# guodashun/peg-in-hole-gym

Hardware: AMD Instinct MI355X
Metric: env-steps/sec (higher is better)
Workload: dtype f32

## Files before the change

### peg_in_hole_gym_amd/csrc/pih_common.h

```cpp
#pragma once
#include <string.h>
#include "../../include/pih.h"
#include "../../include/pih_model.h"
#include "pih_math.h"

namespace pih {

constexpr int NL = PIH_NL, ANL = PIH_ARM_NL, ONL = PIH_OBJ_NL, ND = PIH_NDOF;
constexpr int NSAMP = PIH_PIPE_NSAMP;
constexpr int CMAX = 48;
constexpr int CAMAX = 12;
constexpr int CL = 20;
constexpr int NROWC = 3 * CMAX;
constexpr int WPS = 39;
constexpr int WMS = 31;
constexpr int NMOT = 32;
constexpr int NLIM = 18;
static_assert(PIH_DBG_UDOT + ND <= PIH_DBG_NCONTACT && PIH_DBG_CONTACT + PIH_DBG_CONTACT_STRIDE * CMAX <= PIH_DBG_DINV &&
              PIH_DBG_DINV + 3 * CMAX <= PIH_DBG_CYCLES && PIH_DBG_XCC_ID < PIH_DEBUG_WORDS, "debug words of the peg-in-hole step (include/pih.h PIH_DBG_*) overlap");

PIH_CONST int L_PARENT[NL] = PIH_LINK_PARENT;
PIH_CONST int L_JTYPE[NL] = PIH_LINK_JTYPE;
PIH_CONST real L_RFIX[NL][9] = PIH_LINK_RFIX;
PIH_CONST real L_TFIX[NL][3] = PIH_LINK_TFIX;
PIH_CONST real L_AXIS[NL][3] = PIH_LINK_AXIS;
PIH_CONST real L_MASS[NL] = PIH_LINK_MASS;
PIH_CONST real L_COM[NL][3] = PIH_LINK_COM;
PIH_CONST real L_INERTIA[NL][6] = PIH_LINK_INERTIA;
PIH_CONST real L_LO[NL] = PIH_LINK_LO;
PIH_CONST real L_HI[NL] = PIH_LINK_HI;
PIH_CONST real L_DAMPING[NL] = PIH_LINK_DAMPING;
PIH_CONST real L_MU[NL] = PIH_LINK_MU;
PIH_CONST real ARM_BASE_R[9] = PIH_ARM_BASE_R;
namespace model_ce {
constexpr int JT[NL] = PIH_LINK_JTYPE;
constexpr double DAMP[NL] = PIH_LINK_DAMPING;
constexpr bool structure_ok() {
  for (int L = 0; L < NL; L++) {
    const int want = L < 7 ? PIH_JT_REVOLUTE : (L < ANL ? PIH_JT_PRISMATIC : (L == ANL ? PIH_JT_FLOATING : PIH_JT_REVOLUTE));
    if (JT[L] != want || DAMP[L] != 0.0) return false;
  }
  return true;
}
static_assert(ANL == 9 && structure_ok(), "joint_type() below restates the structure of PIH_LINK_JTYPE / PIH_LINK_DAMPING");
}
PIH_HD int joint_type(int L) { return L < 7 ? PIH_JT_REVOLUTE : (L < ANL ? PIH_JT_PRISMATIC : (L == ANL ? PIH_JT_FLOATING : PIH_JT_REVOLUTE)); }
PIH_CONST real EE_R[9] = PIH_EE_R;
PIH_CONST real EE_T[3] = PIH_EE_T;
PIH_CONST real ARM_REST[9] = PIH_ARM_REST;
PIH_CONST real FBOX_C[2][3] = PIH_FINGER_BOX_C;
PIH_CONST real FBOX_H[3] = PIH_FINGER_BOX_H;
PIH_CONST int ASPH_LINK[PIH_ARM_NSPH] = PIH_ARM_SPH_LINK;
PIH_CONST real ASPH_C[PIH_ARM_NSPH][3] = PIH_ARM_SPH_C;
PIH_CONST real ASPH_R[PIH_ARM_NSPH] = PIH_ARM_SPH_R;
PIH_CONST int SAMP_LINK[NSAMP] = PIH_PIPE_SAMP_LINK;
PIH_CONST real SAMP_Y[NSAMP] = PIH_PIPE_SAMP_Y;
PIH_CONST int SAMP_VERTEX[NSAMP] = PIH_PIPE_SAMP_VERTEX;
PIH_CONST real HOLE_POS[3] = PIH_HOLE_POS;
PIH_CONST real UR5_RFIX[6][9] = PIH_UR5_RFIX;
PIH_CONST real UR5_TFIX[6][3] = PIH_UR5_TFIX;
PIH_CONST real UR5_AXIS[6][3] = PIH_UR5_AXIS;
PIH_CONST real UR5_BASE_T[3] = PIH_UR5_BASE_T;
PIH_CONST real UR5_EE_R[9] = PIH_UR5_EE_R;
PIH_CONST real UR5_EE_T[3] = PIH_UR5_EE_T;
PIH_CONST real IDENT3[9] = {1, 0, 0, 0, 1, 0, 0, 0, 1};
PIH_CONST real ZERO3[3] = {0, 0, 0};
PIH_CONST int FSM_STEPS[10] = PIH_FSM_STEPS;

#define PIH_PI ((real)3.14159265358979323846)
#define PIH_LIN_DAMP ((real)0.04)
#define PIH_ANG_DAMP ((real)0.04)
#define PIH_MAX_COORD_VEL ((real)100)
#define PIH_MAX_FRICTION ((real)10)
#define PIH_BIG ((real)1e30)
#define PIH_MEM_FENCE() __asm__ volatile("" ::: "memory")

#ifdef PIH_AREAL
typedef PIH_AREAL areal;
#else
typedef real areal;
#endif

struct Params {
  real dt, resid, erp, warm, margin, slop, ikdamp, ikres, dv;
  int iters, ikiters, mode, maxsteps, autoreset, selfcol, armcol, debug, env0, pgsmode, attachball, noprio, nospec;
  int object;
  int checkstride;
  uint64_t seed;
};

inline void config_defaults(pih_config* c) {
  memset(c, 0, sizeof *c);
  c->n_envs = 1; c->env_index0 = 0; c->mode = 0; c->solver_iters = 50; c->ik_iters = 20; c->max_episode_steps = 2227; c->auto_reset = 0;
  c->enable_self_collision = 1; c->enable_arm_collision = 3; c->task_id = PIH_TASK_PEG_IN_HOLE; c->debug = 0; c->schedule = 1; c->exit_check_stride = 16;
  c->seed = 0; c->dt = 1.0f / 240.0f; c->residual_threshold = 1e-7f; c->erp = 0.2f; c->warmstart = 0.85f; c->contact_margin = 0.005f;
  c->linear_slop = 1e-5f; c->ik_damping = 0.5f; c->ik_residual = 1e-4f; c->dv = 2.0f / 240.0f;
}
inline Params params_from_config(const pih_config* c) {
  Params P;
  P.dt = (real)c->dt; P.resid = (real)c->residual_threshold; P.erp = (real)c->erp; P.warm = (real)c->warmstart; P.margin = (real)c->contact_margin;
  P.slop = (real)c->linear_slop; P.ikdamp = (real)c->ik_damping; P.ikres = (real)c->ik_residual; P.dv = (real)c->dv;
  P.iters = c->solver_iters; P.ikiters = c->ik_iters; P.mode = c->mode; P.maxsteps = c->max_episode_steps; P.autoreset = c->auto_reset;
  P.selfcol = c->enable_self_collision; P.armcol = c->enable_arm_collision; P.debug = c->debug; P.env0 = c->env_index0; P.seed = c->seed;
  P.pgsmode = c->solver_path; P.attachball = c->attach_ball; P.noprio = (c->schedule & 4) != 0; P.nospec = (c->schedule & 64) != 0;
  P.checkstride = c->exit_check_stride < 1 ? 1 : c->exit_check_stride; P.object = c->object_id;
  return P;
}

template <bool DOUBLED = true, class FC, class FN> PIH_HD int pgs_iteration_loop(int iters, int stride, FC checked, FN unchecked) {
  int it = 0;
  const int lead = stride <= 1 ? iters : 4;
  while (it < iters && it < lead) { it++; if (checked()) return it; }
  while (it < iters) {
    const int stop = it + stride - 1 < iters - 1 ? it + stride - 1 : iters - 1;
    if (DOUBLED) {
      while (it < stop) {
        it++; unchecked();
        if (it >= stop) break;
        it++; unchecked();
      }
    } else {
#pragma nounroll
      while (it < stop) { it++; unchecked(); }
    }
    it++; if (checked()) return it;
  }
  return it;
}

PIH_HD void count_nonfinite_reset(real& rng, real& rng_hi, real& count) {
  rng = (finite_small(rng) && rng >= 0 && rng < (real)16777216) ? rng : (real)0;
  rng_hi = (finite_small(rng_hi) && rng_hi >= 0 && rng_hi < (real)16777216) ? rng_hi : (real)0;
  const real nb = count; count = (finite_small(nb) && nb >= 0 ? nb : (real)0) + 1;
}

PIH_HD int link_dof(int L) { return L < ANL ? L : (L == ANL ? 9 : L + 5); }

constexpr int CREC = 32;
enum : int {
  CR_P = 0,
  CR_LB = 3,
  CR_FLOOR = 4,
  CR_MU = 5,
  CR_ANG = 6,
  CR_PAD = 7,
  CR_DIR0 = 8,
  CR_DINV0 = 11,
  CR_KSTRIDE = 4,
  CR_RHS = 20,
  CR_G = 23,
  CR_LAM = 26,
  CR_DVP_N = CR_LAM,
  CR_THRESH = 29,
  CR_DVP_T1 = CR_THRESH,
};
static_assert(CR_THRESH + 3 == CREC && CR_DINV0 == CR_DIR0 + 3 && CR_DIR0 + 3 * CR_KSTRIDE == CR_RHS && CR_DVP_T1 == CR_DVP_N + 3, "contact record layout");
static_assert(CR_P % 4 == 0 && CR_DIR0 % 4 == 0 && CR_KSTRIDE == 4 && CR_RHS % 4 == 0 && CREC % 4 == 0, "pgs() reads the record as eight real4: (p, lb), (dir k, dinv k) and (rhs, G) each are one 16-byte group");
// ... 523 lines not shown
          else {
            real c = dot(d1, rr);
            if (e <= EPS) { tt = 0; ss = clampr(-c / a, 0, 1); }
            else {
              real b = dot(d1, d2), den = a * e - b * b;
              ss = den > EPS ? clampr((b * f - c * e) / den, 0, 1) : (real)0;
              tt = (b * ss + f) / e;
              if (tt < 0) { tt = 0; ss = clampr(-c / a, 0, 1); } else if (tt > 1) { tt = 1; ss = clampr((b - c) / a, 0, 1); }
            }
          }
          V3 c1 = p1 + ss * d1, c2 = p2 + tt * d2, d = c1 - c2;
          real dist = norm(d); depth = dist - 2 * r;
          if (depth < margin && dist >= (real)1e-9) { n = ((real)1 / dist) * d; p = (real)0.5 * (c1 + c2); valid = true; }
        }
      }
      int slot = w.alloc(valid);
      if (valid && slot < CMAX) emit(slot, ANL + s, ANL + t, 1000 + s * 24 + t, p, n, depth, L_MU[ANL + s] * L_MU[ANL + t]);
    });
  }
  int nc = w.alloc_count(); if (nc > CMAX) nc = CMAX;
  sh.nc = nc; sh.nca = nca;
}

PIH_HD void aba_root_inverse(Shared& sh, const real* Mx, areal* rootp) {
  areal Mq[6][6], Iv[6][6];
  for (int i = 0; i < 6; i++) for (int j = 0; j < 6; j++) { Mq[i][j] = Mx[8 * i + j]; Iv[i][j] = i == j ? (areal)1 : (areal)0; }
#pragma unroll
  for (int k = 0; k < 6; k++) {
    areal pv = (areal)1 / Mq[k][k];
#pragma unroll
    for (int j = 0; j < 6; j++) { Mq[k][j] *= pv; Iv[k][j] *= pv; }
#pragma unroll
    for (int i = 0; i < 6; i++) if (i != k) {
      areal f = Mq[i][k];
#pragma unroll
      for (int j = 0; j < 6; j++) { Mq[i][j] -= f * Mq[k][j]; Iv[i][j] -= f * Iv[k][j]; }
    }
  }
  for (int i = 0; i < 6; i++) { for (int j = 0; j < 6; j++) sh.Inv6[6 * i + j] = (real)Iv[i][j]; rootp[i] = Mx[8 * i + 6]; }
}
PIH_HD int aba_own_word(int i, int j) {
  const int ii = i < 3 ? i : i - 3, jj = j < 3 ? j : j - 3;
  const int sym = ii == jj ? ii : ii + jj + 2;
  if (i >= 6 || j >= 7) return 27;
  if (j == 6) return 21 + i;
  if (i < 3 && j < 3) return sym;
  if (i >= 3 && j >= 3) return 15 + sym;
  if (i < 3) return 6 + 3 * i + jj;
  return 6 + 3 * j + ii;
}
static_assert(NROWC >= 144, "scratch of the inward sweep aliases r_lam");

struct RowOut { real* wa; real* wp; };
PIH_HD real response(const Shared& sh, int la, int lb, V3 p, V3 dir, int jm, RowOut out, V3* dvp_out = nullptr, bool ang = false) {
  real jw = 0; V3 dvp = mk(0, 0, 0);
  bool arm = (la >= 0 && la < ANL) || (lb >= 0 && lb < ANL) || (jm >= 0 && jm < ANL);
  bool obj = (la >= ANL) || (lb >= ANL) || (jm >= ANL);
  if (arm && out.wa) {
    const bool aa_ = la >= 0 && la < ANL, ab_ = lb >= 0 && lb < ANL;
    const V3 rA = p - ld3(sh.LO[aa_ ? la : 0]), rB = p - ld3(sh.LO[ab_ ? lb : 0]);
    const V3 tqa = ang ? dir : cross(rA, dir), tqb = ang ? dir : cross(rB, dir), tl = ang ? mk(0, 0, 0) : dir;
    struct LinkC { V3 a, Ua, Ul, r; real Di; };
    auto linkc = [&](int L) __attribute__((always_inline)) -> LinkC {
      LinkC c; c.a = ld3(sh.LA[L]); c.Ua = ld3(sh.AU[L]); c.Ul = ld3(sh.AU[L] + 3); c.r = ld3(sh.AR[L]); c.Di = sh.ADinv[L]; return c;
    };
    V3 Qa[ANL], Ql[ANL]; real uu[ANL];
#pragma unroll
    for (int L = 0; L < ANL; L++) { Qa[L] = mk(0, 0, 0); Ql[L] = mk(0, 0, 0); }
    LinkC nx = linkc(ANL - 1);
#pragma unroll
    for (int L = ANL - 1; L >= 0; L--) {
      const LinkC c = nx;
      if (L > 0) nx = linkc(L - 1);
      if (L == la) { Qa[L] = Qa[L] + tqa; Ql[L] = Ql[L] + tl; }
      if (L == lb) { Qa[L] = Qa[L] - tqb; Ql[L] = Ql[L] - tl; }
      constexpr int JT[ANL] = {0, 0, 0, 0, 0, 0, 0, 1, 1};
      constexpr int PAR[ANL] = {-1, 0, 1, 2, 3, 4, 5, 6, 6};
      real u = (L == jm ? (real)1 : (real)0) + (JT[L] == 0 ? dot(c.a, Qa[L]) : dot(c.a, Ql[L]));
      uu[L] = u;
      if (PAR[L] >= 0) {
        real ud = u * c.Di;
        V3 qa = Qa[L] - ud * c.Ua, ql = Ql[L] - ud * c.Ul;
        Qa[PAR[L]] = Qa[PAR[L]] + qa + cross(c.r, ql); Ql[PAR[L]] = Ql[PAR[L]] + ql;
      }
      PIH_MEM_FENCE();
    }
    V3 dw[ANL], dvv[ANL]; real wq[ANL];
    nx = linkc(0);
#pragma unroll
    for (int L = 0; L < ANL; L++) {
      const LinkC c = nx;
      if (L + 1 < ANL) nx = linkc(L + 1);
      constexpr int JT[ANL] = {0, 0, 0, 0, 0, 0, 0, 1, 1};
      constexpr int PAR[ANL] = {-1, 0, 1, 2, 3, 4, 5, 6, 6};
      V3 aa = mk(0, 0, 0), ll = mk(0, 0, 0);
      if (PAR[L] >= 0) { aa = dw[PAR[L]]; ll = dvv[PAR[L]] + cross(aa, c.r); }
      real dq = (uu[L] - dot(c.Ua, aa) - dot(c.Ul, ll)) * c.Di;
      if (JT[L] == 0) { dw[L] = aa + dq * c.a; dvv[L] = ll; } else { dw[L] = aa; dvv[L] = ll + dq * c.a; }
      wq[L] = dq;
      if (L == jm) jw += dq;
      if (L == la) dvp = dvp + (ang ? dw[L] : dvv[L] + cross(dw[L], rA));
      if (L == lb) dvp = dvp - (ang ? dw[L] : dvv[L] + cross(dw[L], rB));
      PIH_MEM_FENCE();
    }
#pragma unroll
    for (int L = 0; L < ANL; L++) out.wa[L] = wq[L];
  }
// ... 10 lines not shown
#pragma unroll
    for (int j = ONL - 1; j >= 0; j--) {
      const int L = ANL + j;
      const LinkC c = nx;
      if (j > 1) nx = linkc(L - 1);
      if (L == la) { Qa = Qa + tqa; Ql = Ql + tl; }
      if (L == lb) { Qa = Qa - tqb; Ql = Ql - tl; }
      if (j > 0) {
        real u = (L == jm ? (real)1 : (real)0) + dot(c.a, Qa);
        uu[j] = u;
        real ud = u * c.Di;
        V3 qa = Qa - ud * c.Ua, ql = Ql - ud * c.Ul;
        Qa = qa + cross(c.r, ql); Ql = ql;
      }
      PIH_MEM_FENCE();
    }
    real Q[6] = {Qa.x, Qa.y, Qa.z, Ql.x, Ql.y, Ql.z}, x[6];
#pragma unroll
    for (int i = 0; i < 6; i++) { real s = 0;
#pragma unroll
      for (int k = 0; k < 6; k++) s += sh.Inv6[6 * i + k] * Q[k];
      x[i] = s; }
    V3 dw = mk(x[0], x[1], x[2]), dvv = mk(x[3], x[4], x[5]);
    real wq[5 + ONL];
    wq[0] = dvv.x; wq[1] = dvv.y; wq[2] = dvv.z; wq[3] = dw.x; wq[4] = dw.y; wq[5] = dw.z;
    if (ANL == la) dvp = dvp + (ang ? dw : dvv + cross(dw, rA));
    if (ANL == lb) dvp = dvp - (ang ? dw : dvv + cross(dw, rB));
    nx = linkc(ANL + 1);
#pragma unroll
    for (int j = 1; j < ONL; j++) {
      const int L = ANL + j;
      const LinkC c = nx;
      if (j + 1 < ONL) nx = linkc(L + 1);
      V3 ll = dvv + cross(dw, c.r);
      real dq = (uu[j] - dot(c.Ua, dw) - dot(c.Ul, ll)) * c.Di;
      dw = dw + dq * c.a; dvv = ll;
      wq[5 + j] = dq;
      if (L == jm) jw += dq;
      if (L == la) dvp = dvp + (ang ? dw : dvv + cross(dw, rA));
      if (L == lb) dvp = dvp - (ang ? dw : dvv + cross(dw, rB));
      PIH_MEM_FENCE();
    }
#pragma unroll
    for (int k = 0; k < 5 + ONL; k++) out.wp[k] = wq[k];
  }
  if (dvp_out) *dvp_out = dvp;
  return jw + dot(dir, dvp);
}

PIH_HD V3 point_vel(const Shared& sh, int L, V3 p) { return ld3(sh.VV[L]) + cross(ld3(sh.VW[L]), p - ld3(sh.LO[L])); }

struct MotorW { real w[PIH_OBJ_NJ]; };

template <class W> PIH_HD void build_rows(W& w, Shared& sh, const Params& P, const Ovf& ov, MotorW& mw, bool defer_arm = false) {
  const real dt = P.dt;
  link_velocities(w, sh);
  const int nrows = NMOT + 3 * sh.nc;
  constexpr int FIRST = NMOT + 3 * MERGED_CONTACTS;
#pragma nounroll
  for (int pass = 0; pass < 2; pass++) {
    const int g0 = pass == 0 ? 0 : FIRST, g1 = pass == 0 ? (nrows < FIRST ? nrows : FIRST) : nrows;
    if (g1 > g0) w.par(g1 - g0, [&](int i) {
      const int g = g0 + i;
      const bool ismotor = g < NMOT;
      const int row = ismotor ? 0 : g - NMOT, c = row / 3, k = row - 3 * c;
      int la = -1, lb = -1, jm = -1;
      bool ang = false;
      V3 p = mk(0, 0, 0), dir = mk(0, 0, 0);
      RowOut o; o.wa = nullptr; o.wp = nullptr;
      if (ismotor) {
        jm = g < 9 ? g : ANL + 1 + (g - 9);
        if (g < 9) o.wa = wma_row(sh, g); else o.wp = wmp_row(sh, g - 9);
      } else {
        la = sh.c_la[c]; lb = sh.c_lb[c];
        ang = sh.c_mu[c] < (real)-1.5;
        V3 n = ld3(sh.c_n[c]); p = ld3(sh.c_p[c]);
        V3 t1, t2; plane_space(n, t1, t2);
        dir = k == 0 ? n : (k == 1 ? t1 : t2);
        real* wr = wp_row(sh, ov, row);
        o.wa = wr; o.wp = wr + 9;
        if (!(la < ANL || (lb >= 0 && lb < ANL))) { for (int j = 0; j < 9; j++) wr[j] = 0; }
        if (!(la >= ANL || lb >= ANL)) { for (int j = 9; j < ND; j++) wr[j] = 0; }
        wr[ND] = 0;
      }
      V3 dvp;
      const real jw = response(sh, la, lb, p, dir, jm, o, &dvp, ang);
      const real di = (real)1 / jw;
      if (ismotor) {
        const int d = link_dof(jm);
        sh.mrec[g][MR_DINV] = di; sh.mrec[g][MR_THRESH] = (real)sqrt(P.resid) * di;
        if (!(defer_arm && g < 9)) sh.mrec[g][MR_RHS] = (sh.mrec[g][MR_VT] - sh.u[d]) * di;
        if (g < 9) sh.lrec[g][LR_JW] = jw;
      } else {
        real* R = crec_of(sh, ov, c);
        V3 vr = ang ? ld3(sh.VW[la]) : point_vel(sh, la, p);
        if (lb >= 0) vr = vr - (ang ? ld3(sh.VW[lb]) : point_vel(sh, lb, p));
        real ju = dot(dir, vr);
        real lam = 0, rhs;
        if (k == 0) {
          real pen = sh.c_depth[c] + P.slop;
          real vb = pen > 0 ? -pen / dt : -P.erp * pen / dt;
          if (sh.c_mu[c] < 0) vb = -P.erp * sh.c_depth[c] / dt;
          if (ang) vb = -P.erp * dot(p, dir) / dt;
          rhs = (vb - ju) * di;
          int ncache = (int)sh.S[PIH_S_CACHE_N]; real key = (real)sh.c_key[c];
          for (int q = 0; q < ncache; q++) if (sh.S[PIH_S_CACHE_KEY + q] == key) { lam = P.warm * sh.S[PIH_S_CACHE_LAMBDA + q]; break; }
          const bool bil = sh.c_mu[c] < 0;
          R[CR_P] = p.x; R[CR_P + 1] = p.y; R[CR_P + 2] = p.z; R[CR_LB] = bil ? -PIH_BIG : (real)0; R[CR_FLOOR] = bil ? PIH_BIG : (real)0; R[CR_MU] = sh.c_mu[c]; R[CR_ANG] = ang ? (real)1 : (real)0; R[CR_PAD] = 0;
        } else rhs = ((ang ? -P.erp * dot(p, dir) / dt : (real)0) - ju) * di;
        R[CR_DIR0 + CR_KSTRIDE * k] = dir.x; R[CR_DIR0 + CR_KSTRIDE * k + 1] = dir.y; R[CR_DIR0 + CR_KSTRIDE * k + 2] = dir.z; R[CR_DINV0 + CR_KSTRIDE * k] = di;
        R[CR_RHS + k] = rhs;
        if (k < 2) { R[CR_DVP_N + 3 * k] = dvp.x; R[CR_DVP_N + 3 * k + 1] = dvp.y; R[CR_DVP_N + 3 * k + 2] = dvp.z; }
        sh.r_lam[row] = lam;
      }
    });
    if (pass == 0) {
      w.par(NLIM, [&](int k) {
        int L = k >> 1, side = k & 1;
        real q = sh.S[PIH_S_QARM + L];
        real pen = side == 0 ? q - L_LO[L] : L_HI[L] - q;
        real vb = pen > 0 ? -pen / dt : -P.erp * pen / dt;
        real sg = side == 0 ? (real)1 : (real)-1;
        sh.lrec[L][LR_LO + side] = (vb - sg * sh.u[L]) * sh.mrec[L][MR_DINV];
      });
      pull_motor_rows(w, sh, mw);
    }
  }
  w.par(sh.nc, [&](int c) {
    real* R = crec_of(sh, ov, c);
    V3 t1 = ld3(R + CR_DIR0 + CR_KSTRIDE), t2 = ld3(R + CR_DIR0 + CR_KSTRIDE * 2), dn = ld3(R + CR_DVP_N), d1 = ld3(R + CR_DVP_T1);
    R[CR_G] = dot(t1, dn); R[CR_G + 1] = dot(t2, dn); R[CR_G + 2] = dot(t2, d1);
    R[CR_LAM] = sh.r_lam[3 * c]; R[CR_LAM + 1] = 0; R[CR_LAM + 2] = 0;
    { const real sr = (real)sqrt(P.resid); R[CR_THRESH] = sr * R[CR_DINV0]; R[CR_THRESH + 1] = sr * R[CR_DINV0 + CR_KSTRIDE]; R[CR_THRESH + 2] = sr * R[CR_DINV0 + CR_KSTRIDE * 2]; }
  });
}

struct DofGeom { V3 a, o; int L; int kind; };
PIH_HD DofGeom dof_geom(const Shared& sh, int d) {
  DofGeom g; g.a = mk(0, 0, 0); g.o = mk(0, 0, 0); g.L = 0; g.kind = 2;
  if (d < 9) { g.L = d; g.a = ld3(sh.LA[d]); g.o = ld3(sh.LO[d]); g.kind = d < 7 ? 0 : 1; }
  else if (d < 15) { int k = d - 9; g.L = ANL; g.o = ld3(sh.LO[ANL]); int kk = k % 3; g.a = mk(kk == 0, kk == 1, kk == 2); g.kind = k < 3 ? 1 : 0; }
  else if (d < ND) { g.L = d - 5; g.a = ld3(sh.LA[g.L]); g.o = ld3(sh.LO[g.L]); g.kind = 0; }
  return g;
}
PIH_HD bool is_anc(int L, int X) {
  if (X < 0) return false;
  if (L < ANL) return X < ANL && ((L <= 6 && L <= X) || L == X);
  return X >= ANL && L <= X;
}
PIH_HD real jac_entry(const DofGeom& g, int la, int lb, V3 p, V3 dir, bool ang = false) {
  if (g.kind == 2) return 0;
  real s = (is_anc(g.L, la) ? (real)1 : (real)0) - (is_anc(g.L, lb) ? (real)1 : (real)0);
  if (s == 0) return 0;
  real v = ang ? (g.kind == 0 ? dot(dir, g.a) : (real)0) : (g.kind == 0 ? dot(dir, cross(g.a, p - g.o)) : dot(dir, g.a));
  return s * v;
}

}
```

### peg_in_hole_gym_amd/csrc/pih_hip.hip

```cpp
#include <hip/hip_runtime.h>
#include <dlfcn.h>
#include <cstdio>
#include <cstdlib>
#include <cstring>
#include <string>
#include <vector>
#include "pih_device.h"
#include "pih_render.h"
#include "pih_fly.h"
#include "pih_fly_render.h"

using namespace pih;

namespace pih {
void fly_image_launch(int fmt, dim3 grid, hipStream_t stream, const float* state, void* out, const fly::FlyCam& cam, const float* cam_dev,
                      int n, int object, int env_begin, int W, int H, int rows_per_strip, int flags);
void view_launch(int fmt, dim3 grid, hipStream_t stream, const float* state, void* out, const fly::FlyCam& cam, const float* cam_dev,
                 int env_begin, int W, int H, int rows_per_strip, int flags);
int lit_light_check(const float* words, const char** what);
void lit_launch(bool fly_task, int fmt, dim3 grid, hipStream_t stream, const float* state, void* out, const fly::FlyCam& cam, const float* cam_dev,
                const float* light, const float* light_dev, int n, int object, int env_begin, int W, int H, int rows_per_strip, int flags);
void robot_fk_launch(int robot, bool staged, hipStream_t stream, int n, const float* q, const float* qd, float* out);
void robot_jacobian_launch(int robot, bool staged, hipStream_t stream, int n, const float* q, int frame, const float* local_pos, float* out);
void robot_mass_launch(int robot, bool staged, hipStream_t stream, int n, const float* q, float* out);
// ... 41 lines not shown
}

struct FusedArgs {
  int G, n, epoch;
  const int* bcur; int* bnext; int* bzero;
  float* mail; int* flags; int* err;
};
__device__ __forceinline__ int fused_lookup_env(const int* __restrict__ bcur, int b, int n, int lane) {
  int p = bcur[lane];
#pragma unroll
  for (int d = 1; d < 64; d <<= 1) { const int t = __shfl_up(p, d); if (lane >= d) p += t; }
  const unsigned long long m = __ballot(p > b);
  if (m == 0) return b;
  const int k = __ffsll((long long)m) - 1;
  const int base = k > 0 ? __shfl(p, k - 1) : 0;
  const int e = bcur[64 + (size_t)k * n + (b - base)];
  return e >= 0 && e < n ? e : b;
}

__global__ void __launch_bounds__(64, 2) pih_step_kernel(Params P, float* __restrict__ state, const float* __restrict__ actions,
                                                      float* __restrict__ obs, float* __restrict__ reward,
                                                      unsigned char* __restrict__ done, float* __restrict__ dbg,
                                                      float* __restrict__ ovf, const int* __restrict__ order, FusedArgs F) {
  const int lane = threadIdx.x;
  if ((int)blockIdx.x < F.G) {
    __builtin_amdgcn_s_setprio(3);
    if (blockIdx.x == 0 && F.bzero) F.bzero[lane] = 0;
    const int env = blockIdx.x * 64 + lane;
    if (env < F.n) {
      const float* S = state + (size_t)env * PIH_STATE_WORDS;
      if (P.autoreset || S[PIH_S_DONE] == 0) {
        float a[4] = {0, 0, 0, 0};
        if (actions) { a[0] = actions[env * 4]; a[1] = actions[env * 4 + 1]; a[2] = actions[env * 4 + 2]; a[3] = actions[env * 4 + 3]; }
        const CtrlOut o = controller_compute(S, P, a);
        float* m = F.mail + (size_t)env * CTRL_WORDS;
        const float ov[13] = {o.target[0], o.target[1], o.target[2], o.target[3], o.target[4], o.target[5], o.target[6], o.target[7], o.target[8], o.fsm, o.fsmt, o.grasp_angle, o.attach_qz};
#pragma unroll
        for (int i = 0; i < 13; i++) mail_store(m + i, ov[i]);
      }
    }
    mailbox_publish(F.flags, F.epoch);
    return;
  }
  __shared__ Shared sh;
  const int b = blockIdx.x - F.G;
  const int env = __builtin_amdgcn_readfirstlane(F.bcur ? fused_lookup_env(F.bcur, b, F.n, lane) : (order ? order[b] : b));
  Wave w; w.l = lane; w.counter = 0;
  float* rec = state + (size_t)env * PIH_STATE_WORDS;
#pragma unroll
  for (int i = 0; i < PIH_STATE_WORDS / 64; i++) sh.S[lane + 64 * i] = rec[lane + 64 * i];
  __syncthreads();
  float o[5], r; unsigned char d;
  Ovf ov; ov.base = ovf + (size_t)env * OVF_WORDS;
  w.dbg = dbg ? dbg + (size_t)env * PIH_DEBUG_WORDS : nullptr; w.dbgmode = P.debug; w.prio_on = !P.noprio;
  if (F.G > 0) { w.cflags = F.flags; w.cmail = F.mail; w.cerr = F.err; w.cepoch = F.epoch; w.cenv = env; }
  step_env(w, sh, P, ov, env, nullptr, o, &r, &d, dbg ? dbg + (size_t)env * PIH_DEBUG_WORDS : nullptr);
  __syncthreads();
#pragma unroll
  for (int i = 0; i < PIH_STATE_WORDS / 64; i++) rec[lane + 64 * i] = sh.S[lane + 64 * i];
  if (lane < 5 && obs) obs[env * 5 + lane] = o[0] * (lane == 0) + o[1] * (lane == 1) + o[2] * (lane == 2) + o[3] * (lane == 3) + o[4] * (lane == 4);
  if (lane == 0) {
    if (reward) reward[env] = r; if (done) done[env] = d;
    if (F.bnext) {
      const int bin = contact_bin(sh.S[PIH_S_NCONTACT]);
      const int rnk = atomicAdd(F.bnext + bin, 1);
      if (rnk < F.n) F.bnext[64 + (size_t)bin * F.n + rnk] = env;
    }
  }
}

__global__ void __launch_bounds__(256) pih_bins_init_kernel(const float* __restrict__ state, int* __restrict__ bins, int n) {
  for (int e = blockIdx.x * 256 + threadIdx.x; e < n; e += gridDim.x * 256) {
    const int bin = contact_bin(state[(size_t)e * PIH_STATE_WORDS + PIH_S_NCONTACT]);
    const int rnk = atomicAdd(bins + bin, 1);
    bins[64 + (size_t)bin * n + rnk] = e;
  }
}

__global__ void __launch_bounds__(64) pih_reset_kernel(Params P, float* __restrict__ state, const unsigned char* __restrict__ mask, int hard, int rewind) {
  __shared__ Shared sh;
  const int env = blockIdx.x, lane = threadIdx.x;
  if (mask && !mask[env]) return;
  Wave w; w.l = lane; w.counter = 0;
  float* rec = state + (size_t)env * PIH_STATE_WORDS;
  for (int i = 0; i < PIH_STATE_WORDS / 64; i++) sh.S[lane + 64 * i] = rec[lane + 64 * i];
  __syncthreads();
  if (hard) sh.S[PIH_S_SPARE] = 0;
  if (rewind) { sh.S[PIH_S_RNG] = 0; sh.S[PIH_S_RNG_HI] = 0; }
  __syncthreads();
  reset_state(sh.S, P, P.env0 + env);
  __syncthreads();
  fk_all(w, sh);
  float tip[7]; tip_pose(sh, tip);
  for (int i = 0; i < 7; i++) sh.S[PIH_S_TIP + i] = tip[i];
  V3 ee; M3 eR; ee_pose(sh, ee, eR);
  sh.S[PIH_S_EE] = ee.x + sh.S[PIH_S_OFFSET]; sh.S[PIH_S_EE + 1] = ee.y + sh.S[PIH_S_OFFSET + 1]; sh.S[PIH_S_EE + 2] = ee.z + sh.S[PIH_S_OFFSET + 2];
  __syncthreads();
  for (int i = 0; i < PIH_STATE_WORDS / 64; i++) rec[lane + 64 * i] = sh.S[lane + 64 * i];
}

__global__ void __launch_bounds__(64) pih_init_offsets_kernel(float* __restrict__ state, const float* __restrict__ offsets, int n) {
  int e = blockIdx.x * 64 + threadIdx.x;
  if (e >= n) return;
  float* rec = state + (size_t)e * PIH_STATE_WORDS;
  for (int k = 0; k < 3; k++) rec[PIH_S_OFFSET + k] = offsets ? offsets[3 * e + k] : 0.f;
}

// ... 342 lines not shown
  if (fused) L.grid += L.G;
  return L;
}

static int create_impl(pih_handle* h, const float* offsets_host, float** offd) {
  const pih_config* cfg = &h->cfg;
  size_t nb = (size_t)cfg->n_envs * h->words * sizeof(float);
  HIPCHK(h, hipMalloc(&h->state, nb));
  HIPCHK(h, hipMemset(h->state, 0, nb));
  if (cfg->debug) { HIPCHK(h, hipMalloc(&h->dbg, (size_t)cfg->n_envs * PIH_DEBUG_WORDS * sizeof(float))); HIPCHK(h, hipMemset(h->dbg, 0, (size_t)cfg->n_envs * PIH_DEBUG_WORDS * sizeof(float))); }
  if (offsets_host) {
    HIPCHK(h, hipMalloc(offd, (size_t)cfg->n_envs * 3 * sizeof(float)));
    HIPCHK(h, hipMemcpy(*offd, offsets_host, (size_t)cfg->n_envs * 3 * sizeof(float), hipMemcpyHostToDevice));
  }
  if (h->fly) {
    h->flyquad = (cfg->schedule & 32) == 0;
    int cus = 0; HIPCHK(h, hipDeviceGetAttribute(&cus, hipDeviceAttributeMultiprocessorCount, h->device));
    const FlyLaunch fused = fly_launch(h, true);
    h->fused = (cfg->schedule & 8) == 0 && fused.grid <= fused.per_cu * cus;
    for (const FlyLaunch& L : {fly_launch(h, false), fused})
      HIPCHK(h, hipFuncSetAttribute(reinterpret_cast<const void*>(L.kernel), hipFuncAttributeMaxDynamicSharedMemorySize, (int)L.lds));
    if (h->fused) { int rc = mailbox_alloc(h, (size_t)fused.G * 64 * fly::NJ); if (rc) return rc; }
    const int nb64 = (cfg->n_envs + 63) / 64;
    hipLaunchKernelGGL(pih_fly_init_offsets_kernel, dim3(nb64), dim3(64), 0, 0, h->state, *offd, cfg->n_envs);
    hipLaunchKernelGGL(pih_fly_reset_kernel, dim3(nb64), dim3(64), 0, 0, h->P, h->state, (const unsigned char*)nullptr, 0, 0, cfg->n_envs);
    HIPCHK(h, hipGetLastError());
    HIPCHK(h, hipDeviceSynchronize());
    return 0;
  }
  HIPCHK(h, hipMalloc(&h->ovf, ((size_t)cfg->n_envs * OVF_WORDS + OVF_PAD_WORDS) * sizeof(float)));
  HIPCHK(h, hipMemset(h->ovf, 0, ((size_t)cfg->n_envs * OVF_WORDS + OVF_PAD_WORDS) * sizeof(float)));
  h->fused = (cfg->schedule & 8) == 0;
  if (h->fused) {
    int rc = mailbox_alloc(h, (size_t)cfg->n_envs * CTRL_WORDS);
    if (rc) return rc;
    if (cfg->schedule & 1) {
      h->bin_ints = 64 + (size_t)64 * cfg->n_envs;
      HIPCHK(h, hipMalloc(&h->bins, 3 * h->bin_ints * sizeof(int)));
      HIPCHK(h, hipMemset(h->bins, 0, 3 * h->bin_ints * sizeof(int)));
    }
  } else if (cfg->schedule & 1) HIPCHK(h, hipMalloc(&h->order, (size_t)cfg->n_envs * sizeof(int)));
  hipLaunchKernelGGL(pih_init_offsets_kernel, dim3((cfg->n_envs + 63) / 64), dim3(64), 0, 0, h->state, *offd, cfg->n_envs);
  hipLaunchKernelGGL(pih_reset_kernel, dim3(cfg->n_envs), dim3(64), 0, 0, h->P, h->state, (const unsigned char*)nullptr, 0, 0);
  if (h->bins) hipLaunchKernelGGL(pih_bins_init_kernel, dim3(64), dim3(256), 0, 0, h->state, h->bins + h->bin_ints, cfg->n_envs);
  HIPCHK(h, hipGetLastError());
  HIPCHK(h, hipDeviceSynchronize());
  return 0;
}

int pih_create(const pih_config* cfg, const float* offsets_host, pih_handle** out) {
  if (!cfg || !out || cfg->n_envs <= 0) { g_err = "pih_create: bad arguments"; return -2; }
  if (cfg->task_id != PIH_TASK_PEG_IN_HOLE && cfg->task_id != PIH_TASK_RANDOM_FLY) { g_err = "pih_create: unknown task_id"; return -2; }
  if (cfg->task_id == PIH_TASK_RANDOM_FLY && (cfg->object_id < 0 || cfg->object_id >= PIH_FLY_NOBJ)) { g_err = "pih_create: unknown object_id for the random-fly task"; return -2; }
  if ((cfg->schedule & 3) >= 2 || (cfg->schedule & ~(3 | 4 | 8 | 32 | 64)) != 0) {
    g_err = "pih_create: schedule = " + std::to_string(cfg->schedule) + " is not supported (0 or 1, plus any of 4, 8, 32, 64)";
    return -2;
  }
  int ndev = 0;
  hipError_t e = hipGetDeviceCount(&ndev);
  if (e != hipSuccess || ndev == 0) { g_err = "pih_create: no HIP device (this library has no CPU path)"; return -3; }
  pih_handle* h = new pih_handle;
  h->cfg = *cfg; h->P = params_from_config(cfg);
  h->fly = cfg->task_id == PIH_TASK_RANDOM_FLY; h->words = h->fly ? PIH_FLY_STATE_WORDS : PIH_STATE_WORDS;
  float* offd = nullptr;
  int rc = -1;
  if (hipGetDevice(&h->device) == hipSuccess) rc = create_impl(h, offsets_host, &offd);
  else g_err = "pih_create: hipGetDevice failed";
  if (offd) hipFree(offd);
  if (rc != 0) { pih_destroy(h); return rc; }
  *out = h;
  return 0;
}

int pih_reset(pih_handle* h, const uint8_t* mask_dev, int hard, uint64_t seed, void* stream) {
  if (!h) return -2;
  if (mask_dev && (seed != 0 || h->rewind_pending)) {
    h->err = "pih_reset: a new seed (seed != 0, or a pending pih_reseed) needs a reset of all envs (mask_dev = NULL)";
    return -2;
  }
  PIH_ENTER(h);
  RoctxRange range(h->cfg.debug != 0, hard ? "pih_reset(hard)" : "pih_reset");
  if (seed != 0) { h->cfg.seed = seed; h->P.seed = seed; h->rewind_pending = true; }
  const int rewind = h->rewind_pending ? 1 : 0;
  h->rewind_pending = false;
  if (h->fly) hipLaunchKernelGGL(pih_fly_reset_kernel, dim3((h->cfg.n_envs + 63) / 64), dim3(64), 0, (hipStream_t)stream, h->P, h->state, mask_dev, hard != 0, rewind, h->cfg.n_envs);
  else hipLaunchKernelGGL(pih_reset_kernel, dim3(h->cfg.n_envs), dim3(64), 0, (hipStream_t)stream, h->P, h->state, mask_dev, hard != 0, rewind);
  HIPCHK(h, hipGetLastError());
  return 0;
}

int pih_reseed(pih_handle* h, uint64_t seed) {
  if (!h) return -2;
  h->cfg.seed = seed; h->P.seed = seed; h->rewind_pending = true;
  return 0;
}

static int launch_step(pih_handle* h, const float* actions, float* obs, float* reward, uint8_t* done, hipStream_t s) {
  RoctxRange range(h->cfg.debug != 0, h->fly ? "pih_step(random-fly)" : "pih_step(peg-in-hole)");
  EvTriple* t = nullptr;
  if (h->timing > 0 && (h->timing_tick++ % (unsigned)h->timing) == 0) {
    if (h->ev_used == EV_POOL) { int r = drain_events(h); if (r) return r; }
    if (h->ev_used == h->ev.size()) {
      EvTriple n;
      HIPCHK(h, hipEventCreate(&n.a)); HIPCHK(h, hipEventCreate(&n.b)); HIPCHK(h, hipEventCreate(&n.c));
      h->ev.push_back(n);
    }
    t = &h->ev[h->ev_used++];
    HIPCHK(h, hipEventRecord(t->a, s));
// ... 366 lines not shown
```

### peg_in_hole_gym_amd/csrc/pih_wave.h

```cpp
#pragma once
#include <type_traits>
#include "pih_common.h"
#include "pih_mailbox.h"

namespace pih {

PIH_HD void debug_store_time(real* dbg, int at, long long t) { dbg[at] = (real)(t & 0xFFFF); dbg[at + 1] = (real)((t >> 16) & 0xFFFF); dbg[at + 2] = (real)((t >> 32) & 0xFFFF); }
PIH_HD void debug_store_hw_id(real* dbg) { dbg[PIH_DBG_HW_ID] = (real)(__builtin_amdgcn_s_getreg((15 << 11) | 4) & 0xFFFF); dbg[PIH_DBG_XCC_ID] = (real)__builtin_amdgcn_s_getreg((3 << 11) | 20); }

struct Wave {
  int l;
  int counter;
  static constexpr bool controller_inline = false;
  real* dbg = nullptr; int dbgmode = 0; long long t0 = 0, t1 = 0;
  PIH_HD void stamp(int k) { if (dbg && dbgmode == 2) { long long t = __builtin_readcyclecounter(); if (l == 0) dbg[PIH_DBG_CYCLES + k] = (real)(t - t0); t0 = t; } }
  PIH_HD void trace(int at, long long t) { if (l != 0) return; debug_store_time(dbg, at, t); if (at == PIH_DBG_T_START) debug_store_hw_id(dbg); }
  PIH_HD void phase_begin() { if (dbg && dbgmode == 2) { t1 = __builtin_readcyclecounter(); trace(PIH_DBG_T_START, (long long)__builtin_amdgcn_s_memrealtime()); } }
  PIH_HD void phase(int k) { if (dbg && dbgmode == 2) { long long t = __builtin_readcyclecounter(); if (l == 0) dbg[PIH_DBG_CYCLES + k] = (real)(t - t1); t1 = t; if (k == 7) trace(PIH_DBG_T_END, (long long)__builtin_amdgcn_s_memrealtime()); } }
  PIH_HD int lane() const { return l; }
  bool prio_on = true;
  PIH_HD void priority(int contacts) {
    if (!prio_on) return;
    if (contacts > 20) __builtin_amdgcn_s_setprio(3);
    else if (contacts > 14) __builtin_amdgcn_s_setprio(2);
    else if (contacts > 10) __builtin_amdgcn_s_setprio(1);
    else __builtin_amdgcn_s_setprio(0);
  }
  const int* cflags = nullptr; const real* cmail = nullptr; int* cerr = nullptr; int cepoch = 0, cenv = 0;
  PIH_HD void await_controller(Shared& sh) {
    if (!cmail) return;
    mailbox_await(cflags + (cenv >> 6), cepoch, cerr, l == 0);
    __syncthreads();
    if (l < 13) {
      const real v = mail_load(cmail + (size_t)cenv * CTRL_WORDS + l);
      const int word = l < 9 ? PIH_S_TARGET + l : (l == 9 ? (int)PIH_S_FSM : l == 10 ? (int)PIH_S_FSMT : l == 11 ? (int)PIH_S_GRASP_ANGLE : (int)PIH_S_ATTACH_QZ);
      sh.S[word] = v;
    }
    __syncthreads();
  }
  PIH_HD void sync() { __syncthreads(); }
  template <class F> PIH_HD void par(int n, F f) {
    __syncthreads();
    for (int b = 0; b < n; b += 64) { int i = b + l; if (i < n) f(i); }
    __syncthreads();
  }
  template <class F> PIH_HD void par_all(int n, F f) {
    __syncthreads();
    for (int b = 0; b < n; b += 64) { int i = b + l; f(i, i < n); }
    __syncthreads();
  }
  PIH_HD void alloc_reset(int base) { counter = base; }
  PIH_HD int alloc_count() const { return counter; }
  PIH_HD int alloc(bool valid) {
    unsigned long long m = __ballot(valid);
    int slot = counter + __popcll(m & ((1ull << l) - 1ull));
    counter += __popcll(m);
    return valid ? slot : -1;
  }
};
typedef unsigned long long pk2;
PIH_HD pk2 pk_pack(real x, real y) { return (pk2)__builtin_bit_cast(unsigned, x) | ((pk2)__builtin_bit_cast(unsigned, y) << 32); }
PIH_HD real pk_lo(pk2 v) { return __builtin_bit_cast(float, (unsigned)v); }
PIH_HD real pk_hi(pk2 v) { return __builtin_bit_cast(float, (unsigned)(v >> 32)); }
PIH_HD void pk_fma_lo(pk2& acc, pk2 j, pk2 w2) { __asm__("v_pk_fma_f32 %0, %1, %2, %0 op_sel_hi:[1,0,1]" : "+v"(acc) : "v"(j), "v"(w2)); }
PIH_HD void pk_fma_hi(pk2& acc, pk2 j, pk2 w2) { __asm__("v_pk_fma_f32 %0, %1, %2, %0 op_sel:[0,1,0] op_sel_hi:[1,1,1]" : "+v"(acc) : "v"(j), "v"(w2)); }
PIH_HD real rdlane(real v, int lane) {
  return __builtin_bit_cast(float, __builtin_amdgcn_readlane(__builtin_bit_cast(int, v), lane));
}
PIH_HD void gs_row2_normal(pk2& zz, real z, pk2 col, real lo, real& lam, int G, real& dl, real& s0) {
  real cand; unsigned long long m;
  __asm__ volatile("v_max_f32 %0, %6, %7\n\tv_sub_f32 %1, %0, %3\n\tv_readlane_b32 %2, %0, %9\n\tv_readlane_b32 s100, %1, %9\n\t"
                   "s_lshl_b64 %4, 1, %9\n\tv_cndmask_b32_e64 %3, %3, %0, %4\n\tv_pk_fma_f32 %5, s[100:101], %8, %5 op_sel_hi:[0,1,1]"
                   : "=&v"(cand), "=&v"(dl), "=&s"(s0), "+v"(lam), "=&s"(m), "+v"(zz) : "v"(z), "v"(lo), "v"(col), "n"(G) : "scc", "s100", "s101");
}
PIH_HD void gs_row2_bounded(pk2& zz, real z, pk2 col, real hi, real& lam, int G, real& dl) {
  real cand; unsigned long long m;
  __asm__ volatile("v_med3_f32 %0, %5, -%6, %6\n\tv_sub_f32 %1, %0, %2\n\ts_lshl_b64 %3, 1, %8\n\tv_readlane_b32 s100, %1, %8\n\t"
                   "v_cndmask_b32_e64 %2, %2, %0, %3\n\ts_nop 0\n\tv_pk_fma_f32 %4, s[100:101], %7, %4 op_sel_hi:[0,1,1]"
                   : "=&v"(cand), "=&v"(dl), "+v"(lam), "=&s"(m), "+v"(zz) : "v"(z), "v"(hi), "v"(col), "n"(G) : "scc", "s100", "s101");
}
PIH_HD void gs_row2_friction(pk2& zz, real z, pk2 col, real h, real& lam, int G, real& dl) {
  real cand; unsigned long long m;
  __asm__ volatile("v_med3_f32 %0, %5, -%6, %6\n\tv_sub_f32 %1, %0, %2\n\ts_lshl_b64 %3, 1, %8\n\tv_readlane_b32 s100, %1, %8\n\t"
                   "v_cndmask_b32_e64 %2, %2, %0, %3\n\ts_nop 0\n\tv_pk_fma_f32 %4, s[100:101], %7, %4 op_sel_hi:[0,1,1]"
                   : "=&v"(cand), "=&v"(dl), "+v"(lam), "=&s"(m), "+v"(zz) : "v"(z), "v"(h), "v"(col), "n"(G) : "scc", "s100", "s101");
}
PIH_HD void gs_row1_normal(real& z, real b, real lo, real& lam, int G, real& dl, real& s0) {
  real cand, sdl; unsigned long long m;
  __asm__ volatile("v_max_f32 %0, %6, %7\n\tv_sub_f32 %1, %0, %4\n\tv_readlane_b32 %3, %0, %9\n\tv_readlane_b32 %2, %1, %9\n\t"
                   "s_lshl_b64 %5, 1, %9\n\tv_cndmask_b32_e64 %4, %4, %0, %5\n\tv_fmac_f32 %6, %2, %8"
                   : "=&v"(cand), "=&v"(dl), "=&s"(sdl), "=&s"(s0), "+v"(lam), "=&s"(m), "+v"(z) : "v"(lo), "v"(b), "n"(G) : "scc");
}
PIH_HD void gs_row1_friction2(real& z, real b1, real b2, real h, real& lam, int G1, int G2, real& dl1, real& dl2) {
  real cand, sdl; unsigned long long m;
  __asm__ volatile("v_med3_f32 %0, %6, -%7, %7\n\tv_sub_f32 %1, %0, %4\n\ts_lshl_b64 %5, 1, %10\n\tv_readlane_b32 %3, %1, %10\n\t"
                   "v_cndmask_b32_e64 %4, %4, %0, %5\n\ts_nop 0\n\tv_fmac_f32 %6, %3, %8\n\t"
                   "v_med3_f32 %0, %6, -%7, %7\n\tv_sub_f32 %2, %0, %4\n\ts_lshl_b64 %5, 1, %11\n\tv_readlane_b32 %3, %2, %11\n\t"
                   "v_cndmask_b32_e64 %4, %4, %0, %5\n\ts_nop 0\n\tv_fmac_f32 %6, %3, %9"
                   : "=&v"(cand), "=&v"(dl1), "=&v"(dl2), "=&s"(sdl), "+v"(lam), "=&s"(m), "+v"(z) : "v"(h), "v"(b1), "v"(b2), "n"(G1), "n"(G2) : "scc");
}
template <int CTRL> PIH_HD real dpp_add(real x) {
  return x + __builtin_bit_cast(float, __builtin_amdgcn_update_dpp(0, __builtin_bit_cast(int, x), CTRL, 0xF, 0xF, true));
}
PIH_HD real sum8(real x) {
  x = dpp_add<0xB1>(x);
  x = dpp_add<0x4E>(x);
  return dpp_add<0x141>(x);
}
PIH_HD real from_lane(real v, int byte_addr) {
  return __builtin_bit_cast(float, __builtin_amdgcn_ds_bpermute(byte_addr, __builtin_bit_cast(int, v)));
}
PIH_HD int lane_byte(int lane) { return 4 * lane; }
// ... 432 lines not shown
  }
  w.sync();
  return it;
}

PIH_HD int pgs_rows2(Wave& w, Shared& sh, const Params& P, const Ovf& ov, const MotorW& mw) {
  const int nc = __builtin_amdgcn_readfirstlane(sh.nc);
  w.sync();
  const int lane = w.lane();
  constexpr int D = 12;
  real* const Bg = ov.base + OVF_B_OFF + 2 * lane;
  static_assert(OVF_MW_WORDS + OVF_PAD_WORDS >= D * 128, "the ring reads D columns past the streamed-column area");
  const unsigned l8 = (unsigned)lane * 8u;
  struct RowC { real di, rhs, thr, lb, ub, mu, fl, lam0; };
  auto rowconst = [&](int g) __attribute__((always_inline)) -> RowC {
    RowC r; r.di = 0; r.rhs = 0; r.thr = PIH_BIG; r.lb = 0; r.ub = 0; r.mu = 0; r.fl = 0; r.lam0 = 0;
    if (g < 9) r.di = sh.mrec[g][MR_DINV];
    else if (g < NMOT) { r.di = sh.mrec[g][MR_DINV]; r.rhs = sh.mrec[g][MR_RHS]; r.thr = sh.mrec[g][MR_THRESH]; r.ub = sh.mrec[g][MR_IMP]; r.lb = -r.ub; }
    else {
      const int row = g - NMOT, c = row / 3, k = row - 3 * c;
      if (c < nc) {
        const real* R = crec_of(sh, ov, c);
        r.di = R[CR_DINV0 + CR_KSTRIDE * k]; r.rhs = R[CR_RHS + k]; r.thr = R[CR_THRESH + k]; r.mu = R[CR_MU]; r.fl = R[CR_FLOOR];
        if (k == 0) { r.lb = R[CR_LB]; r.ub = PIH_BIG; r.lam0 = sh.r_lam[3 * c]; }
      }
    }
    return r;
  };
  const RowC c0 = rowconst(lane), c1 = rowconst(64 + lane);
  pk2 BB[KREG];
  {
    const int row0 = lane - NMOT, row1 = 32 + lane;
    const real* w0 = row0 >= 0 && row0 < 3 * nc ? wp_row(sh, ov, row0) : nullptr;
    const real* w1 = row1 < 3 * nc ? wp_row(sh, ov, row1) : nullptr;
#pragma unroll
    for (int m = 0; m < NMOT; m++) {
      const int dm = m < 9 ? m : 15 + (m - 9);
      real a0;
      if (m < 9) a0 = lane < 9 ? mw.w[m] : (real)0;
      else {
        const real up = __builtin_bit_cast(float, __builtin_amdgcn_ds_bpermute(4 * ((lane + 6) & 63), __builtin_bit_cast(int, mw.w[m - 9])));
        a0 = (lane >= 9 && lane < NMOT) ? up : (real)0;
      }
      if (w0) a0 = w0[dm];
      const real a1 = w1 ? w1[dm] : (real)0;
      BB[m] = pk_pack(((lane == m && m >= 9) ? (real)1 : (real)0) - c0.di * a0, -c1.di * a1);
    }
  }
  real* const Mg = ov.base + OVF_MW_OFF + lane;
#pragma unroll
  for (int j = 0; j < PIH_OBJ_NJ; j++) Mg[j * 64] = mw.w[j];
  pk2 JJ[ND];
  {
    auto geom = [&](int g, int& la, int& lb, V3& p, V3& dir, bool& ang, bool& live) __attribute__((always_inline)) {
      la = -1; lb = -1; p = mk(0, 0, 0); dir = mk(0, 0, 0); ang = false; live = false;
      if (g < NMOT) return;
      const int row = g - NMOT, c = row / 3, k = row - 3 * c;
      if (c >= nc) return;
      live = true; la = sh.c_la[c]; lb = sh.c_lb[c];
      const real* R = crec_of(sh, ov, c);
      p = ld3(R + CR_P); dir = ld3(R + CR_DIR0 + CR_KSTRIDE * k); ang = R[CR_ANG] != 0;
    };
    int la0, lb0, la1, lb1; V3 p0, d0, p1, d1; bool a0, a1, l0, l1;
    geom(lane, la0, lb0, p0, d0, a0, l0); geom(64 + lane, la1, lb1, p1, d1, a1, l1);
    const int md = lane < 9 ? lane : 15 + (lane - 9);
    DofGeom gn = dof_geom(sh, 0);
#pragma unroll
    for (int d = 0; d < ND; d++) {
      const DofGeom g = gn;
      if (d + 1 < ND) gn = dof_geom(sh, d + 1);
      real j0 = lane < NMOT ? (d == md ? (real)1 : (real)0) : (l0 ? jac_entry(g, la0, lb0, p0, d0, a0) : (real)0);
      real j1 = l1 ? jac_entry(g, la1, lb1, p1, d1, a1) : (real)0;
      __asm__ volatile("" : "+v"(j0), "+v"(j1) :: "memory");
      JJ[d] = pk_pack(j0, j1);
    }
  }
  w.sync();
  static_assert(ND % 2 == 0 && KREG == NMOT, "entries are consumed in pairs; every contact column is streamed");
  real wv0 = 0, wv1 = 0;
  auto column = [&](int cb, auto pairof) __attribute__((always_inline)) {
    pk2 acc[3] = {0, 0, 0};
    constexpr int NB = (ND + 3) / 4;
    pk2 wq[2][6];
    auto request = [&](int blk, pk2* q) __attribute__((always_inline)) {
#pragma unroll
      for (int h = 0; h < 2; h++)
#pragma unroll
        for (int k = 0; k < 3; k++) { const int d = 4 * blk + 2 * h; q[3 * h + k] = d < ND ? pairof(k * WPS + d) : (pk2)0; }
    };
    request(0, wq[0]);
#pragma unroll
    for (int blk = 0; blk < NB; blk++) {
      if (blk + 1 < NB) request(blk + 1, wq[(blk + 1) & 1]);
      __asm__ volatile("" ::: "memory");
#pragma unroll
      for (int h = 0; h < 2; h++) {
        const int d = 4 * blk + 2 * h;
        if (d < ND) {
#pragma unroll
          for (int k = 0; k < 3; k++) { pk_fma_lo(acc[k], JJ[d], wq[blk & 1][3 * h + k]); pk_fma_hi(acc[k], JJ[d + 1], wq[blk & 1][3 * h + k]); }
        }
      }
    }
#pragma unroll
    for (int k = 0; k < 3; k++) {
      const int i = NMOT + 3 * cb + k;
      const real b0 = (lane == i ? (real)1 : (real)0) - c0.di * pk_lo(acc[k]), b1 = (64 + lane == i ? (real)1 : (real)0) - c1.di * pk_hi(acc[k]);
      Bg[(size_t)(i - KREG) * 128] = b0; Bg[(size_t)(i - KREG) * 128 + 1] = b1;
      if (k == 0) { const real l = sh.r_lam[3 * cb]; wv0 += b0 * l; wv1 += b1 * l; }
    }
  };
  {
    const int nl = nc < CL ? nc : CL;
#pragma unroll 1
    for (int cb = 0; cb < nl; cb++) {
      const real* wr = sh.b.Wp[3 * cb];
      column(cb, [&](int o) __attribute__((always_inline)) { return pk_pack(wr[o], wr[o + 1]); });
    }
    typedef const real __attribute__((address_space(1)))* grp;
#pragma unroll 1
    for (int cb = CL; cb < nc; cb++) {
      const grp wr = (grp)(ov.base + (size_t)(3 * (cb - CL)) * WPS);
      column(cb, [&](int o) __attribute__((always_inline)) { return pk_pack(wr[o], wr[o + 1]); });
    }
  }
#pragma unroll
  for (int q = NMOT; q < KREG; q++) if (q >= NMOT + 3 * nc) BB[q] = 0;
  unsigned angmask = 0;
// ... 279 lines not shown
```

Baseline: 11.77 million.

## Specialize row response and Jacobian build for single-body contacts and arm-free frames

Adds a wave-wide check for whether any contact row involves a second body. When none does, row response and Jacobian entries are built with single-body templates. The Jacobian build now uses per-DOF compile-time specialization (jac_entry_flat via static_for) and skips the arm DOF block when no arm contacts exist. A schedule bit (256) forces the two-body path. The cost is extra code size and register pressure from two instantiated paths, and a ballot per pass.

```diff
diff --git a/peg_in_hole_gym_amd/csrc/pih_common.h b/peg_in_hole_gym_amd/csrc/pih_common.h
--- a/peg_in_hole_gym_amd/csrc/pih_common.h
+++ b/peg_in_hole_gym_amd/csrc/pih_common.h
@@ -1,4 +1,5 @@
 #pragma once
+#include <type_traits>
 #include <string.h>
 #include "../../include/pih.h"
 #include "../../include/pih_model.h"
@@ -81,6 +82,8 @@
 typedef real areal;
 #endif
 
+enum { STEPSW_NOPRIO = 1,
+       STEPSW_TWOBODY = 2 };
 struct Params {
   real dt, resid, erp, warm, margin, slop, ikdamp, ikres, dv;
   int iters, ikiters, mode, maxsteps, autoreset, selfcol, armcol, debug, env0, pgsmode, attachball, noprio, nospec;
@@ -102,7 +105,7 @@
   P.slop = (real)c->linear_slop; P.ikdamp = (real)c->ik_damping; P.ikres = (real)c->ik_residual; P.dv = (real)c->dv;
   P.iters = c->solver_iters; P.ikiters = c->ik_iters; P.mode = c->mode; P.maxsteps = c->max_episode_steps; P.autoreset = c->auto_reset;
   P.selfcol = c->enable_self_collision; P.armcol = c->enable_arm_collision; P.debug = c->debug; P.env0 = c->env_index0; P.seed = c->seed;
-  P.pgsmode = c->solver_path; P.attachball = c->attach_ball; P.noprio = (c->schedule & 4) != 0; P.nospec = (c->schedule & 64) != 0;
+  P.pgsmode = c->solver_path; P.attachball = c->attach_ball; P.noprio = ((c->schedule & 4) ? STEPSW_NOPRIO : 0) | ((c->schedule & 256) ? STEPSW_TWOBODY : 0); P.nospec = (c->schedule & 64) != 0;
   P.checkstride = c->exit_check_stride < 1 ? 1 : c->exit_check_stride; P.object = c->object_id;
   return P;
 }
@@ -732,7 +735,9 @@
 static_assert(NROWC >= 144, "scratch of the inward sweep aliases r_lam");
 
 struct RowOut { real* wa; real* wp; };
-PIH_HD real response(const Shared& sh, int la, int lb, V3 p, V3 dir, int jm, RowOut out, V3* dvp_out = nullptr, bool ang = false) {
+template <bool TWO_BODY = true>
+PIH_HD real response(const Shared& sh, int la, int lb_row, V3 p, V3 dir, int jm, RowOut out, V3* dvp_out = nullptr, bool ang = false) {
+  const int lb = TWO_BODY ? lb_row : -1;
   real jw = 0; V3 dvp = mk(0, 0, 0);
   bool arm = (la >= 0 && la < ANL) || (lb >= 0 && lb < ANL) || (jm >= 0 && jm < ANL);
   bool obj = (la >= ANL) || (lb >= ANL) || (jm >= ANL);
@@ -849,6 +854,8 @@
 
 struct MotorW { real w[PIH_OBJ_NJ]; };
 
+template <class W, class F> PIH_HD bool wave_any(W&, int n0, int n1, F f) { for (int i = n0; i < n1; i++) if (f(i)) return true; return false; }
+
 template <class W> PIH_HD void build_rows(W& w, Shared& sh, const Params& P, const Ovf& ov, MotorW& mw, bool defer_arm = false) {
   const real dt = P.dt;
   link_velocities(w, sh);
@@ -857,6 +864,8 @@
 #pragma nounroll
   for (int pass = 0; pass < 2; pass++) {
     const int g0 = pass == 0 ? 0 : FIRST, g1 = pass == 0 ? (nrows < FIRST ? nrows : FIRST) : nrows;
+    const int c0 = pass == 0 ? 0 : MERGED_CONTACTS, c1 = pass == 0 ? (sh.nc < MERGED_CONTACTS ? sh.nc : MERGED_CONTACTS) : sh.nc;
+    const bool two = (P.noprio & STEPSW_TWOBODY) != 0 || wave_any(w, c0, c1, [&](int c) { return sh.c_lb[c] >= 0; });
     if (g1 > g0) w.par(g1 - g0, [&](int i) {
       const int g = g0 + i;
       const bool ismotor = g < NMOT;
@@ -881,7 +890,7 @@
         wr[ND] = 0;
       }
       V3 dvp;
-      const real jw = response(sh, la, lb, p, dir, jm, o, &dvp, ang);
+      const real jw = two ? response<true>(sh, la, lb, p, dir, jm, o, &dvp, ang) : response<false>(sh, la, lb, p, dir, jm, o, &dvp, ang);
       const real di = (real)1 / jw;
       if (ismotor) {
         const int d = link_dof(jm);
@@ -952,5 +961,23 @@
   real v = ang ? (g.kind == 0 ? dot(dir, g.a) : (real)0) : (g.kind == 0 ? dot(dir, cross(g.a, p - g.o)) : dot(dir, g.a));
   return s * v;
 }
-
-}
+template <int D, bool TWO_BODY> PIH_HD real jac_entry_flat(const DofGeom& g, int la, int lb, V3 p, V3 dir, bool ang) {
+  static_assert(D >= 0 && D < ND, "a DOF");
+  constexpr int L = D < 9 ? D : (D < 15 ? ANL : D - 5);
+  constexpr bool REV = D < 9 ? D < 7 : (D < 15 ? D >= 12 : true);
+  auto anc = [&](int X) -> bool { return L < ANL ? (L <= 6 ? (X >= L) & (X < ANL) : X == L) : X >= L; };
+  const bool sa = anc(la), sb = TWO_BODY ? anc(lb) : false;
+  real v;
+  if (REV) {
+    const V3 c = cross(g.a, p - g.o);
+    v = dot(dir, mk(ang ? g.a.x : c.x, ang ? g.a.y : c.y, ang ? g.a.z : c.z));
+  } else {
+    const real t = dot(dir, g.a);
+    v = ang ? (real)0 : t;
+  }
+  const real sv = TWO_BODY ? (sa ? v : -v) : v;
+  return sa != sb ? sv : (real)0;
+}
+template <int I0, int I1, class F> PIH_HD void static_for(F& f) { if constexpr (I0 < I1) { f(std::integral_constant<int, I0>()); static_for<I0 + 1, I1>(f); } }
+
+}
diff --git a/peg_in_hole_gym_amd/csrc/pih_hip.hip b/peg_in_hole_gym_amd/csrc/pih_hip.hip
--- a/peg_in_hole_gym_amd/csrc/pih_hip.hip
+++ b/peg_in_hole_gym_amd/csrc/pih_hip.hip
@@ -117,7 +117,7 @@
   __syncthreads();
   float o[5], r; unsigned char d;
   Ovf ov; ov.base = ovf + (size_t)env * OVF_WORDS;
-  w.dbg = dbg ? dbg + (size_t)env * PIH_DEBUG_WORDS : nullptr; w.dbgmode = P.debug; w.prio_on = !P.noprio;
+  w.dbg = dbg ? dbg + (size_t)env * PIH_DEBUG_WORDS : nullptr; w.dbgmode = P.debug; w.prio_on = !(P.noprio & STEPSW_NOPRIO);
   if (F.G > 0) { w.cflags = F.flags; w.cmail = F.mail; w.cerr = F.err; w.cepoch = F.epoch; w.cenv = env; }
   step_env(w, sh, P, ov, env, nullptr, o, &r, &d, dbg ? dbg + (size_t)env * PIH_DEBUG_WORDS : nullptr);
   __syncthreads();
@@ -566,8 +566,8 @@
   if (!cfg || !out || cfg->n_envs <= 0) { g_err = "pih_create: bad arguments"; return -2; }
   if (cfg->task_id != PIH_TASK_PEG_IN_HOLE && cfg->task_id != PIH_TASK_RANDOM_FLY) { g_err = "pih_create: unknown task_id"; return -2; }
   if (cfg->task_id == PIH_TASK_RANDOM_FLY && (cfg->object_id < 0 || cfg->object_id >= PIH_FLY_NOBJ)) { g_err = "pih_create: unknown object_id for the random-fly task"; return -2; }
-  if ((cfg->schedule & 3) >= 2 || (cfg->schedule & ~(3 | 4 | 8 | 32 | 64)) != 0) {
-    g_err = "pih_create: schedule = " + std::to_string(cfg->schedule) + " is not supported (0 or 1, plus any of 4, 8, 32, 64)";
+  if ((cfg->schedule & 3) >= 2 || (cfg->schedule & ~(3 | 4 | 8 | 32 | 64 | 256)) != 0) {
+    g_err = "pih_create: schedule = " + std::to_string(cfg->schedule) + " is not supported (0 or 1, plus any of 4, 8, 32, 64, 256)";
     return -2;
   }
   int ndev = 0;
diff --git a/peg_in_hole_gym_amd/csrc/pih_wave.h b/peg_in_hole_gym_amd/csrc/pih_wave.h
--- a/peg_in_hole_gym_amd/csrc/pih_wave.h
+++ b/peg_in_hole_gym_amd/csrc/pih_wave.h
@@ -58,6 +58,11 @@
     return valid ? slot : -1;
   }
 };
+template <class F> PIH_HD bool wave_any(Wave& w, int n0, int n1, F f) {
+  unsigned long long m = 0;
+  for (int b = n0; b < n1; b += 64) { const int i = b + w.l; m |= __ballot(i < n1 && f(i)); }
+  return m != 0;
+}
 typedef unsigned long long pk2;
 PIH_HD pk2 pk_pack(real x, real y) { return (pk2)__builtin_bit_cast(unsigned, x) | ((pk2)__builtin_bit_cast(unsigned, y) << 32); }
 PIH_HD real pk_lo(pk2 v) { return __builtin_bit_cast(float, (unsigned)v); }
@@ -596,28 +601,40 @@
   for (int j = 0; j < PIH_OBJ_NJ; j++) Mg[j * 64] = mw.w[j];
   pk2 JJ[ND];
   {
-    auto geom = [&](int g, int& la, int& lb, V3& p, V3& dir, bool& ang, bool& live) __attribute__((always_inline)) {
-      la = -1; lb = -1; p = mk(0, 0, 0); dir = mk(0, 0, 0); ang = false; live = false;
+    auto geom = [&](int g, int& la, int& lb, V3& p, V3& dir, bool& ang) __attribute__((always_inline)) {
+      la = -1; lb = -1; p = mk(0, 0, 0); dir = mk(0, 0, 0); ang = false;
       if (g < NMOT) return;
       const int row = g - NMOT, c = row / 3, k = row - 3 * c;
       if (c >= nc) return;
-      live = true; la = sh.c_la[c]; lb = sh.c_lb[c];
+      la = sh.c_la[c]; lb = sh.c_lb[c];
       const real* R = crec_of(sh, ov, c);
       p = ld3(R + CR_P); dir = ld3(R + CR_DIR0 + CR_KSTRIDE * k); ang = R[CR_ANG] != 0;
     };
-    int la0, lb0, la1, lb1; V3 p0, d0, p1, d1; bool a0, a1, l0, l1;
-    geom(lane, la0, lb0, p0, d0, a0, l0); geom(64 + lane, la1, lb1, p1, d1, a1, l1);
+    int la0, lb0, la1, lb1; V3 p0, d0, p1, d1; bool a0, a1;
+    geom(lane, la0, lb0, p0, d0, a0); geom(64 + lane, la1, lb1, p1, d1, a1);
     const int md = lane < 9 ? lane : 15 + (lane - 9);
-    DofGeom gn = dof_geom(sh, 0);
-#pragma unroll
-    for (int d = 0; d < ND; d++) {
-      const DofGeom g = gn;
-      if (d + 1 < ND) gn = dof_geom(sh, d + 1);
-      real j0 = lane < NMOT ? (d == md ? (real)1 : (real)0) : (l0 ? jac_entry(g, la0, lb0, p0, d0, a0) : (real)0);
-      real j1 = l1 ? jac_entry(g, la1, lb1, p1, d1, a1) : (real)0;
-      __asm__ volatile("" : "+v"(j0), "+v"(j1) :: "memory");
-      JJ[d] = pk_pack(j0, j1);
-    }
+    const bool hasarm = __builtin_amdgcn_readfirstlane(sh.nca) != 0;
+    if (!hasarm) {
+#pragma unroll
+      for (int d = 0; d < 9; d++) JJ[d] = pk_pack(lane < NMOT && d == md ? (real)1 : (real)0, (real)0);
+    }
+    const bool two = (P.noprio & STEPSW_TWOBODY) != 0 || __ballot(lb0 >= 0 || lb1 >= 0) != 0;
+    auto jrows = [&](auto TWOTAG) __attribute__((always_inline)) {
+      constexpr bool TWO = decltype(TWOTAG)::value;
+      DofGeom gn;
+      auto entry = [&](auto DT) __attribute__((always_inline)) {
+        constexpr int d = decltype(DT)::value;
+        const DofGeom g = gn;
+        if (d + 1 < ND) gn = dof_geom(sh, d + 1);
+        real j0 = lane < NMOT ? (d == md ? (real)1 : (real)0) : jac_entry_flat<d, TWO>(g, la0, lb0, p0, d0, a0);
+        real j1 = jac_entry_flat<d, TWO>(g, la1, lb1, p1, d1, a1);
+        __asm__ volatile("" : "+v"(j0), "+v"(j1) :: "memory");
+        JJ[d] = pk_pack(j0, j1);
+      };
+      if (hasarm) { gn = dof_geom(sh, 0); static_for<0, 9>(entry); } else gn = dof_geom(sh, 9);
+      static_for<9, ND>(entry);
+    };
+    if (two) jrows(std::true_type()); else jrows(std::false_type());
   }
   w.sync();
   static_assert(ND % 2 == 0 && KREG == NMOT, "entries are consumed in pairs; every contact column is streamed");
```

Result: no change. 11.83 million, median of 6 (+0.5%).
